# Tariq-Abuhashim/semantic-slam

Measured on AMD Instinct MI355X. Metric: Mvoxels/sec integrated, 512³ grid @ 640×480 depth; achieved HBM GB/s %peak, higher is better.
Workload: dtype f32

## Files before the change

include/tsdf_hip_diag.h:

```cpp
#ifndef TSDF_HIP_DIAG_H
#define TSDF_HIP_DIAG_H

#include "tsdf_hip.h"

#ifdef __cplusplus
extern "C" {
#endif


int tsdf_integrate_sequence_timed(tsdf_volume *vol, const float *depth_dev, const float *cam2world,
                                  int32_t n_frames, float *elapsed_ms);

int tsdf_integrate_frames_timed(tsdf_volume *vol, const float *const *depth_dev, const uint8_t *const *masks_dev,
                                const float *cam2world, int32_t n_frames, float *elapsed_ms);


int tsdf_probe_graph_replay(tsdf_volume *vol, const float *depth_dev, const float *cam2world, int32_t n_frames,
                            int32_t iters, float *ms_launches, float *ms_graph);

int tsdf_probe_stream(tsdf_volume *vol, int32_t non_temporal, int32_t n_iters, float *elapsed_ms);


int tsdf_selftest_fastdiv(int32_t device, uint64_t seed, uint64_t n_samples, float fx, float cx,
                          uint64_t *mismatches, float first_bad[4]);

int tsdf_selftest_fastdiv_band(int32_t device, uint64_t seed, uint64_t n_samples, uint64_t *mismatches,
                               float first_bad[4]);

int tsdf_selftest_round(int32_t device, uint64_t *mismatches, float first_bad[4]);

int tsdf_selftest_tile_tables(int32_t device, const float *depth_dev, const uint8_t *mask_dev, int32_t im_height,
                              int32_t im_width, float max_depth, uint64_t *mismatches);


int32_t tsdf_frames_per_launch(const tsdf_volume *vol);
int tsdf_shortcut_stats(tsdf_volume *vol, int32_t enable, uint64_t counts_out[3]);
int tsdf_brick_list_stats(tsdf_volume *vol, uint64_t counts_out[4]);
int tsdf_classification_info(tsdf_volume *vol, double info_out[2]);

int tsdf_store_stats(tsdf_volume *vol, int64_t out[9]);

int tsdf_last_cam2base(const tsdf_volume *vol, float out[16]);


int tsdf_set_kernel_variant(tsdf_volume *vol, int32_t variant);

int tsdf_set_brick_shape(tsdf_volume *vol, int32_t quads, int32_t rows, int32_t slices);
int tsdf_brick_shape(const tsdf_volume *vol, int32_t shape_out[3]);
int tsdf_default_brick_shape(const tsdf_config *cfg, int32_t shape_out[3]);

#ifdef __cplusplus
}
#endif
#endif
```

semantic_slam_amd/capi.py:

```python
import ctypes as C
import os

import numpy as np

_PKG = os.path.dirname(os.path.abspath(__file__))
LIB_PATH = os.environ.get("TSDF_HIP_LIB") or os.path.join(_PKG, "libtsdf_hip.so")

ABI_SYMBOLS = [
    "tsdf_config_default", "tsdf_create", "tsdf_destroy", "tsdf_reset", "tsdf_integrate",
    "tsdf_integrate_u16", "tsdf_convert_depth_u16", "tsdf_set_deferral",
    "tsdf_integrate_device", "tsdf_integrate_cam2base", "tsdf_integrate_masked_device",
    "tsdf_integrate_frames_device",
    "tsdf_sync", "tsdf_download", "tsdf_copy_slices", "tsdf_upload", "tsdf_refresh_summary", "tsdf_device_ptrs", "tsdf_slab_voxels", "tsdf_frames_per_launch", "tsdf_shortcut_stats", "tsdf_brick_list_stats", "tsdf_classification_info", "tsdf_store_stats",
    "tsdf_get_config", "tsdf_last_cam2base", "tsdf_set_stream", "tsdf_get_stream",
    "tsdf_count_surface", "tsdf_extract_surface", "tsdf_extract_crossings", "tsdf_extract_mesh", "tsdf_save_mesh_ply", "tsdf_save_mesh_welded_ply", "tsdf_save_ply", "tsdf_save_bin", "tsdf_load_bin", "tsdf_save_state", "tsdf_load_state",
    "tsdf_integrate_sequence_timed", "tsdf_integrate_frames_timed", "tsdf_probe_graph_replay", "tsdf_probe_stream", "tsdf_selftest_fastdiv", "tsdf_selftest_fastdiv_band", "tsdf_selftest_round", "tsdf_selftest_tile_tables", "tsdf_set_kernel_variant", "tsdf_set_brick_shape", "tsdf_brick_shape", "tsdf_default_brick_shape", "tsdf_last_error",
    "tsdf_version", "tsdf_multiply_matrix", "tsdf_invert_matrix",
    "tsdf_labels_enable", "tsdf_compose_labels", "tsdf_integrate_labels_device", "tsdf_integrate_frames_labels_device",
    "tsdf_download_labels",
    "tsdf_colour_enable", "tsdf_integrate_colour_device", "tsdf_integrate_rgbd", "tsdf_download_colour",
    "tsdf_raycast_params_default", "tsdf_raycast_device", "tsdf_raycast", "tsdf_batch_raycast_device",
    "tsdf_track_params_default", "tsdf_track", "tsdf_track_system",
    "tsdf_batch_track", "tsdf_batch_track_system", "tsdf_track_member_systems",
    "tsdf_fuse_params_default", "tsdf_fuse_volume",
    "tsdf_extent_params_default", "tsdf_volume_extent", "tsdf_batch_extents", "tsdf_group_extent", "tsdf_extent_combine",
    "tsdf_extent_metric", "tsdf_extent_regrid",
    "tsdf_associate_params_default", "tsdf_associate_count", "tsdf_associate_assign", "tsdf_batch_associate",
    "tsdf_segment_params_default", "tsdf_segmenter_create", "tsdf_segmenter_destroy", "tsdf_segmenter_set_stream",
    "tsdf_segment_depth_device", "tsdf_segment_refine_masks_device", "tsdf_segment_frame",
    "tsdf_object_origin", "tsdf_batch_create", "tsdf_batch_destroy", "tsdf_batch_size", "tsdf_batch_volume",
    "tsdf_batch_integrate_device", "tsdf_batch_sync",
    "tsdf_group_create", "tsdf_group_destroy", "tsdf_group_size", "tsdf_group_voxels", "tsdf_group_volume",
    "tsdf_group_integrate", "tsdf_group_integrate_frames", "tsdf_group_set_deferral", "tsdf_group_sync", "tsdf_group_reset", "tsdf_group_download",
    "tsdf_group_extract_surface", "tsdf_group_extract_crossings", "tsdf_group_extract_mesh",
    "tsdf_group_save_ply", "tsdf_group_save_mesh_ply", "tsdf_group_save_bin",
]
DIAG_SYMBOLS = [
    "tsdf_integrate_sequence_timed", "tsdf_integrate_frames_timed",
    "tsdf_probe_graph_replay", "tsdf_probe_stream",
    "tsdf_selftest_fastdiv", "tsdf_selftest_fastdiv_band", "tsdf_selftest_round", "tsdf_selftest_tile_tables",
    "tsdf_shortcut_stats", "tsdf_brick_list_stats", "tsdf_classification_info", "tsdf_store_stats", "tsdf_frames_per_launch", "tsdf_last_cam2base",
    "tsdf_set_kernel_variant", "tsdf_set_brick_shape", "tsdf_brick_shape", "tsdf_default_brick_shape",
]


class TsdfError(RuntimeError):
    pass


SHIPPED_VARIANTS = (0, 1, 3, 7, 8)


def experiments_build():
    return b"+experiments" in load().tsdf_version()


def variants(*wanted):
    exp = experiments_build()
    return [v for v in wanted if v in SHIPPED_VARIANTS or exp]


class TsdfConfig(C.Structure):
    _fields_ = [
        ("im_height", C.c_int32), ("im_width", C.c_int32),
# ... 108 lines not shown
    L.tsdf_integrate.argtypes = [vp, vp, vp]
    L.tsdf_set_deferral.argtypes = [vp, C.c_int32]
    L.tsdf_integrate_u16.argtypes = [vp, vp, C.c_float, C.c_int32, C.c_int32, vp]
    L.tsdf_convert_depth_u16.argtypes = [vp, vp, vp, C.c_float, C.c_int32, C.c_int32]
    L.tsdf_integrate_device.argtypes = [vp, vp, vp]
    L.tsdf_integrate_cam2base.argtypes = [vp, vp, vp]
    L.tsdf_integrate_masked_device.argtypes = [vp, vp, vp, vp]
    L.tsdf_integrate_frames_device.argtypes = [vp, vp, vp, vp, C.c_int32]
    L.tsdf_sync.argtypes = [vp]
    L.tsdf_download.argtypes = [vp, vp, vp]
    L.tsdf_upload.argtypes = [vp, vp, vp]
    L.tsdf_copy_slices.argtypes = [vp, C.c_int32, C.c_int32, vp, vp]
    L.tsdf_refresh_summary.argtypes = [vp]
    L.tsdf_device_ptrs.argtypes = [vp, C.POINTER(vp), C.POINTER(vp)]
    L.tsdf_slab_voxels.argtypes = [vp]
    L.tsdf_slab_voxels.restype = C.c_int64
    L.tsdf_frames_per_launch.argtypes = [vp]
    L.tsdf_frames_per_launch.restype = C.c_int32
    L.tsdf_shortcut_stats.argtypes = [vp, C.c_int32, vp]
    L.tsdf_classification_info.argtypes = [vp, vp]
    L.tsdf_brick_list_stats.argtypes = [vp, vp]
    if hasattr(L, "tsdf_store_stats"):
        L.tsdf_store_stats.argtypes = [vp, i64p]
    L.tsdf_get_config.argtypes = [vp, C.POINTER(TsdfConfig)]
    L.tsdf_last_cam2base.argtypes = [vp, vp]
    L.tsdf_set_stream.argtypes = [vp, vp]
    L.tsdf_get_stream.argtypes = [vp, C.POINTER(vp)]
    L.tsdf_count_surface.argtypes = [vp, C.c_float, i64p]
    L.tsdf_extract_surface.argtypes = [vp, C.c_float, vp, C.c_int64, i64p]
    L.tsdf_extract_crossings.argtypes = [vp, vp, vp, C.c_float, vp, C.c_int64, i64p]
    L.tsdf_extract_mesh.argtypes = [vp, vp, vp, C.c_float, vp, C.c_int64, i64p]
    L.tsdf_save_mesh_ply.argtypes = [vp, C.c_char_p, C.c_float]
    L.tsdf_save_mesh_welded_ply.argtypes = [vp, C.c_char_p, C.c_float]
    L.tsdf_save_ply.argtypes = [vp, C.c_char_p, C.c_float]
    L.tsdf_save_bin.argtypes = [vp, C.c_char_p]
    L.tsdf_load_bin.argtypes = [vp, C.c_char_p]
    L.tsdf_save_state.argtypes = [vp, C.c_char_p]
    L.tsdf_load_state.argtypes = [vp, C.c_char_p]
    L.tsdf_integrate_sequence_timed.argtypes = [vp, vp, vp, C.c_int32, f32p]
    L.tsdf_integrate_frames_timed.argtypes = [vp, vp, vp, vp, C.c_int32, f32p]
    L.tsdf_probe_graph_replay.argtypes = [vp, vp, vp, C.c_int32, C.c_int32, f32p, f32p]
    L.tsdf_probe_stream.argtypes = [vp, C.c_int32, C.c_int32, f32p]
    L.tsdf_selftest_fastdiv.argtypes = [C.c_int32, C.c_uint64, C.c_uint64, C.c_float, C.c_float, C.POINTER(C.c_uint64), f32p]
    L.tsdf_selftest_fastdiv_band.argtypes = [C.c_int32, C.c_uint64, C.c_uint64, C.POINTER(C.c_uint64), f32p]
    L.tsdf_selftest_round.argtypes = [C.c_int32, C.POINTER(C.c_uint64), f32p]
    L.tsdf_selftest_tile_tables.argtypes = [C.c_int32, vp, vp, C.c_int32, C.c_int32, C.c_float, C.POINTER(C.c_uint64)]
# ... 352 lines not shown
    def n_voxels(self):
        return int(self.lib.tsdf_slab_voxels(self._h))

    def shortcut_stats(self, enable=True):
        out = (C.c_uint64 * 3)()
        check(self.lib.tsdf_shortcut_stats(self._h, 1 if enable else 0, out), "tsdf_shortcut_stats")
        return tuple(int(x) for x in out)

    def brick_list_stats(self):
        out = (C.c_uint64 * 4)()
        check(self.lib.tsdf_brick_list_stats(self._h, out), "tsdf_brick_list_stats")
        return tuple(int(x) for x in out)

    def classification_info(self):
        out = (C.c_double * 2)()
        check(self.lib.tsdf_classification_info(self._h, out), "tsdf_classification_info")
        return float(out[0]), int(out[1])

    def store_stats(self):
        out = (C.c_int64 * 9)()
        check(self.lib.tsdf_store_stats(self._h, out), "tsdf_store_stats")
        return {name: tuple(int(x) for x in out[3 * k:3 * k + 3]) for k, name in enumerate(("frames", "masks", "tables"))}

    @property
    def frames_per_launch(self):
        return int(self.lib.tsdf_frames_per_launch(self._h))

    @property
    def slab_shape(self):
        c = self.cfg
        return (c.z_end - c.z_begin, c.dim_y, c.dim_x)

    def device_ptrs(self):
        t, w = C.c_void_p(), C.c_void_p()
        check(self.lib.tsdf_device_ptrs(self._h, C.byref(t), C.byref(w)), "tsdf_device_ptrs")
        return t.value, w.value

    def integrate(self, depth_host, cam2world):
        d = _f32(depth_host, self.cfg.im_height * self.cfg.im_width)
        p = _f32(cam2world, 16)
        check(self.lib.tsdf_integrate(self._h, d.ctypes.data, p.ctypes.data), "tsdf_integrate")

    def set_deferral(self, n_frames):
        check(self.lib.tsdf_set_deferral(self._h, n_frames), "tsdf_set_deferral")

    def integrate_u16(self, raw_u16, cam2world, depth_factor=5000.0, row_step=1, col_step=1):
# ... 490 lines not shown
```

semantic_slam_amd/csrc/host_derive.h:

```cpp
#pragma once
#include <algorithm>
#include <cmath>
#include <cstddef>
#include <cstdint>

#include "tsdf_hip.h"

namespace tsdf_host {

inline bool brick_shape_ok(const tsdf_config &c, int q, int r, int s)
{
    return c.dim_x % 4 == 0 && q >= 1 && r >= 1 && s >= 1 && q * r * s <= 64 && (c.dim_x / 4) % q == 0 &&
           (long long)s * c.dim_x * c.dim_y < (1ll << 30);
}

inline void choose_brick_default(const tsdf_config &c, int &bq, int &br, int &bs)
{
    bq = 0; br = 0; bs = 1;
    if (c.dim_x % 4 != 0) return;
    const int quads = c.dim_x / 4;
    const int nz = c.z_end - c.z_begin;
    double best = 1e300;
    for (int q = 1; q <= 64 && q <= quads; ++q) {
        if (quads % q) continue;
// ... 138 lines not shown
constexpr int64_t kWindowBytes = 512ll << 20;

struct SweepWindow { int cache_lo, cache_hi; };

inline SweepWindow sweep_window(int nz, int dim_x, int dim_y, int64_t window_bytes, bool reverse)
{
    const int64_t slice_bytes = 8 * (int64_t)dim_x * dim_y;
    const int w = (int)std::min<int64_t>(nz, window_bytes / slice_bytes);
    return reverse ? SweepWindow{0, w} : SweepWindow{nz - w, nz};
}

inline bool batch_defers(int members, int64_t total_voxels) { return 2 * (int64_t)members < 10 + total_voxels / 1000000; }

constexpr int64_t kBatchMinVoxelsPerMember = 2000000;
inline bool batch_classifies(Classify mode, int members, int64_t launch_voxels)
{
    const bool big_enough = mode == Classify::Always || launch_voxels >= (int64_t)members * kBatchMinVoxelsPerMember;
    return big_enough && classify_one_frame(mode, launch_voxels);
}

constexpr int kBatchSideStreams = 4;
inline int batch_lanes(int members) { return members < 8 ? 1 : kBatchSideStreams; }

struct Regions {
    size_t add(size_t bytes) { const size_t at = (end_ + 255) / 256 * 256; end_ = at + bytes; return at; }
    size_t total() const { return end_; }
    size_t end_ = 0;
};

}
```

semantic_slam_amd/csrc/tsdf_capi.hip:

```cpp
#include "../../include/tsdf_hip.h"
#include "../../include/tsdf_hip_diag.h"

#include <hip/hip_runtime.h>

#include <algorithm>
#include <cmath>
#include <cstdarg>
#include <cstdio>
#include <cstdlib>
#include <cstring>
#include <new>
#include <string>
#include <vector>

#include "pose_math.h"
#include "host_derive.h"
#include "host_copy.h"
#include "hip_owned.h"
#include "frame_store.h"
#include "tsdf_kernels.hip.h"
#include "tsdf_multiframe.hip.h"
#include "tsdf_labels.hip.h"
#include "tsdf_colour.hip.h"
#include "tsdf_extract.hip.h"
// ... 76 lines not shown
    struct tsdf_group *group_owner = nullptr;
    bool in_flush = false;
    float pend_c2b[16 * tsdfk::kMaxFramesPerLaunch] = {};
    const uint8_t *pend_mask[tsdfk::kMaxFramesPerLaunch] = {};
    int variant = 0;
    int sweep_parity = 0;
#ifdef TSDF_EXPERIMENTS
    StageRing<Staged<tsdfk::FramePose>, kStageSlots> frames;
#endif
    DevPtr<uint16_t> d_label;
    DevPtr<float> d_fp, d_bp;
    float prob_thd = 0.0f;
    DevPtr<uint32_t> d_colour;
    StageRing<Staged<uint8_t>, kStageSlots> rgb;
    DevPtr<uint32_t> d_flags;
    size_t n_flags = 0;
    int nseg = 0;
    int chunks_per_slice = 0;
    bool flat = false;
    int brick_q = 0, brick_r = 0, brick_s = 0;
    int tile = 0;
    bool fine_tables = false;
    bool flags_known_zero = false;
#ifdef TSDF_EXPERIMENTS
    DevBuf<unsigned int> d_super;
#endif
    DevBuf<uint4> d_work;
    int64_t work_nsuper = 0, work_bucket_supers = 0;
    int work_wedge_mode = -1;
    DevPtr<unsigned int> d_shortcut_stats;
    DevPtr<unsigned long long> d_claims;
    HostPtr<unsigned long long> h_claims;
    Event claims_done;
    Stream pre_stream, rb_stream;
    int rb_parity = -1;
    Event pre_done[2], list_free[2], seq_ready;
    int list_parity = 0;
    bool list_used[2] = {false, false};
    bool pipeline_ok = false;
    bool claims_pending = false, claims_known = false;
    double claims_total = 0.0;
    double claim_fraction = 0.0;
    int launches_unclassified = 0;
    DevBuf<char> d_scratch;
    DevBuf<uint8_t> d_wg_class;
    DevBuf<char> d_list;
// ... 229 lines not shown
            const int strips = ((p.tiles_w + 3) / 4) * p.tiles_h;
            hipLaunchKernelGGL(tsdfk::depth_tile_summary<16>, dim3((unsigned)((strips + 3) / 4), m), dim3(64, 4), 0, stream, tp);
        } else {
            const int strips = ((p.tiles_w + 7) / 8) * p.tiles_h;
            hipLaunchKernelGGL(tsdfk::depth_tile_summary<8>, dim3((unsigned)((strips + 3) / 4), m), dim3(64, 4), 0, stream, tp);
        }
        if (p.tiles_w * p.tiles_h <= tsdfk::kTileLdsEntries) {
            const unsigned threads = (p.tiles_w * p.tiles_h > 2048 && !beside_a_launch) ? 1024 : 256;
            const unsigned fine_blocks = fine ? ((unsigned)(p.fine_w * p.fine_h) + threads - 1) / threads : 0u;
            hipLaunchKernelGGL(tsdfk::tile_sparse_table, dim3((unsigned)tsdf_host::tile_levels(p.tiles_w) + fine_blocks, m), dim3(threads), 0, stream, tp.tiles,
                               p.tiles_w, p.tiles_h, k == 0 ? zero_me : (unsigned long long *)nullptr, fine, p.fine_w, p.fine_h);
        } else {
            if (zero_me && k == 0) HIP_TRY(hipMemsetAsync(zero_me, 0, tsdfk::kCounterBytes, stream));
            hipLaunchKernelGGL(tsdfk::tile_sparse_table_scan, dim3((unsigned)tsdf_host::tile_levels(p.tiles_w), m), dim3(256), 0, stream, tp.tiles,
                               p.tiles_w, p.tiles_h);
            if (fine)
                hipLaunchKernelGGL(tsdfk::fine_tile_levels, dim3((unsigned)((p.fine_w * p.fine_h + 255) / 256), m), dim3(256), 0, stream, fine, p.fine_w, p.fine_h);
        }
    }
    HIP_TRY(hipGetLastError());
    return TSDF_OK;
}

int launch_masked_bricks(tsdf_volume *v, tsdfk::IntegrateParams &p)
{
    const int blocks = (p.brick_groups * p.bricks_per_group + 3) / 4, nz = (p.nz + p.brick_s - 1) / p.brick_s;
    StoreSlot table;
    int rc0 = table.take(v, &v->store->tables, v->stream);
    if (rc0) return rc0;
    const size_t n_bricks = (size_t)blocks * nz * 4;
    HIP_TRY(v->d_wg_class.ensure(n_bricks));
    const float *d = p.depth;
    const uint8_t *m = p.mask;
    int rc = build_tile_tables(v->stream, v->cfg, p, &d, &m, 1, table.as<float2>());
    if (rc) return rc;
    tsdfk::FramePose pose;
    pose_from_params(pose, p);
    pose.tiles = table.as<float2>();
    hipLaunchKernelGGL(tsdfk::classify_bricks, dim3((unsigned)((n_bricks + 255) / 256)), dim3(256), 0, v->stream, p, pose,
                       v->d_wg_class, blocks, nz);
    p.wg_class = v->d_wg_class;
    hipLaunchKernelGGL((tsdfk::integrate_single_bricks<kBrickNT>), dim3(blocks, 1, nz), dim3(64, 4, 1), 0, v->stream, p, pose);
    HIP_TRY(hipGetLastError());
    return table.release();
}

int drop_summary(tsdf_volume *v)
{
    if (v->flags_known_zero || v->n_flags == 0) return TSDF_OK;
    HIP_TRY(hipMemsetAsync(v->d_flags, 0, v->n_flags * sizeof(uint32_t), v->stream));
    v->flags_known_zero = true;
    return TSDF_OK;
}

int rebuild_summary(tsdf_volume *v)
{
    if (v->n_flags == 0 || v->n_vox == 0) return TSDF_OK;
    const int nz = v->cfg.z_end - v->cfg.z_begin;
    const int qps = (int)((int64_t)v->cfg.dim_x * v->cfg.dim_y / 4);
    dim3 block(64, 4, 1), grid((v->chunks_per_slice + 3) / 4, 1, nz);
    hipLaunchKernelGGL(tsdfk::recompute_flags, grid, block, 0, v->stream, v->d_tsdf, v->d_weight, v->d_flags, qps,
                       v->chunks_per_slice);
    HIP_TRY(hipGetLastError());
    v->flags_known_zero = false;
    return TSDF_OK;
}

int launch_multi(tsdf_volume *v, const float *const *depth_dev, const uint8_t *const *masks_dev, const float *c2b, int n,
                 const uint16_t *const *label_ims = nullptr, const float *const *score_ims = nullptr, hipEvent_t inputs_ready = nullptr);

double claims_read_back(const tsdf_volume *v)
{
    double claimed = 0.0;
    for (int b = 0; b < tsdfk::kListBuckets; ++b) {
        const unsigned long long w = v->h_claims[(size_t)b * (tsdfk::kBucketStride / sizeof(unsigned long long)) + 1];
        claimed += (double)(w >> 32) + (double)(w & 0xffffffffull);
    }
    return v->claims_total > 0 ? claimed / v->claims_total : 0.0;
}

#ifdef TSDF_EXPERIMENTS
tsdf_host::Variant experiment_variant(int variant);
void experiment_adjust(const tsdf_volume *v, bool labels, bool *classify, int *z_fastest);
int launch_integrate_experiment(tsdf_volume *v, const float *depth_dev, const uint8_t *mask_dev, const float *c2b);
int launch_multi_experiment(tsdf_volume *v, tsdfk::MultiParamsInline &mi, const float *const *depth_dev, const uint8_t *const *masks_dev,
                            const float *c2b, int n, bool labels, bool any_mask, bool classify, bool *handled, double *claims_total);
bool experiment_takes_multi(const tsdf_volume *v, bool labels, bool classify);
// ... 43 lines not shown
        const tsdfk::IntegrateParams p = make_params(v, depth_dev, mask_dev, c2b, 1);
        dim3 block(64, 4, 1), grid((c.dim_x + 63) / 64, (c.dim_y + 3) / 4, nz);
        if (mask_dev) hipLaunchKernelGGL((tsdfk::integrate_scalar<true>), grid, block, 0, v->stream, p);
        else hipLaunchKernelGGL((tsdfk::integrate_scalar<false>), grid, block, 0, v->stream, p);
        HIP_TRY(hipGetLastError());
        return TSDF_OK;
    }
    if (v->flat) {
        return launch_multi(v, &depth_dev, mask_dev ? &mask_dev : nullptr, c2b, 1);
    }
    tsdfk::IntegrateParams p = make_params(v, depth_dev, mask_dev, c2b, 4);
    v->flags_known_zero = false;
    const dim3 block(64, 4, 1), grid((p.xgroups + 63) / 64, (p.dim_y + 7) / 8, p.nz);
    if (mask_dev) {
        const bool classify = tsdf_host::classify_one_frame(var.classify, v->n_vox) && tiles_fit(p.tiles_w, p.tiles_h);
        if (classify && p.brick_q > 0 && (!kExperiments || v->variant != 11)) {
            int rc = launch_masked_bricks(v, p);
            if (rc) return rc;
        } else {
#ifdef TSDF_EXPERIMENTS
            if (v->variant == 11 && classify) return launch_integrate_experiment(v, depth_dev, mask_dev, c2b);
#endif
            set_sweep(v, p);
            hipLaunchKernelGGL((tsdfk::integrate_tile<2, true>), grid, block, 0, v->stream, p);
        }
    } else {
        set_sweep(v, p);
        hipLaunchKernelGGL((tsdfk::integrate_tile<2, false>), grid, block, 0, v->stream, p);
    }
    HIP_TRY(hipGetLastError());
    return TSDF_OK;
}

void compose_cam2base(const tsdf_volume *v, const float *cam2world, float *c2b)
{
    tsdf_host::multiply_matrix(v->base2world_inv, cam2world, c2b);
}

int launch_multi(tsdf_volume *v, const float *const *depth_dev, const uint8_t *const *masks_dev,
                 const float *c2b, int n, const uint16_t *const *label_ims, const float *const *score_ims, hipEvent_t inputs_ready)
{
    const tsdf_config &c = v->cfg;
    const int nz = c.z_end - c.z_begin;
    if (nz == 0 || n == 0) return TSDF_OK;
    auto fill_pose = [&](tsdfk::FramePose &fp, int f) {
        pose_from_params(fp, make_params(v, depth_dev[f], masks_dev ? masks_dev[f] : nullptr, c2b + 16 * f, 4));
        fp.label_im = label_ims ? label_ims[f] : nullptr;
        fp.score_im = label_ims ? score_ims[f] : nullptr;
    };
    const dim3 block(64, 4, 1);
    if (n == 1 && !label_ims) {
        tsdfk::IntegrateParams common = make_params(v, depth_dev[0], nullptr, c2b, 4);
        tsdfk::FramePose pose;
        fill_pose(pose, 0);
        std::memcpy(v->last_cam2base, c2b, sizeof v->last_cam2base);
        v->flags_known_zero = false;
#ifdef TSDF_EXPERIMENTS
        {
            bool handled = false;
            int rc = launch_single_experiment(v, common, pose, depth_dev[0], c2b, &handled);
            if (rc || handled) return rc;
        }
#endif
        if (v->flat && pose.mask != nullptr && tsdf_host::classify_one_frame(variant_of(v->variant).classify, v->n_vox) &&
            tiles_fit(common.tiles_w, common.tiles_h) && common.brick_q > 0) {
            tsdfk::IntegrateParams cp = make_params(v, depth_dev[0], pose.mask, c2b, 4);
            return launch_masked_bricks(v, cp);
// ... 373 lines not shown
    rc = frame.release();
    store_next_pass(v);
    return rc;
}

int apply_host_frame(tsdf_volume *v, StoreSlot &frame, const float cam2world[16], bool defer, bool copies_marked, const uint8_t *rgb_dev = nullptr)
{
    StoreSlot no_mask;
    if (defer) return pool_slot_commit(v, frame, no_mask, cam2world);
    if (!copies_marked) HIP_TRY(hipEventRecord(v->pend_copied, v->copy_stream));
    HIP_TRY(hipStreamWaitEvent(v->stream, v->pend_copied, 0));
    return launch_staged_frame(v, frame, cam2world, rgb_dev);
}

int fill(tsdf_volume *v)
{
    if (v->n_vox == 0) return TSDF_OK;
    size_t n = (size_t)v->n_vox;
    int blocks = (int)std::min<size_t>((n / 4 + 255) / 256, 256 * 8);
    if (blocks < 1) blocks = 1;
    hipLaunchKernelGGL(tsdfk::fill_grid, dim3(blocks), dim3(256), 0, v->stream, v->d_tsdf, v->d_weight, n);
    HIP_TRY(hipGetLastError());
    if (v->n_flags) {
        HIP_TRY(hipMemsetD32Async((hipDeviceptr_t)v->d_flags, 3, v->n_flags, v->stream));
        v->flags_known_zero = false;
    }
    return TSDF_OK;
}

#ifdef TSDF_EXPERIMENTS
#include "tsdf_experiments_host.hip.h"
#endif

}

extern "C" {

const char *tsdf_last_error(void) { return g_last_error.c_str(); }

const char *tsdf_version(void)
{
    return kExperiments ? "tsdf_hip 0.3 (gfx950) +experiments" : "tsdf_hip 0.3 (gfx950)";
}

void tsdf_multiply_matrix(const float a[16], const float b[16], float out[16])
{
    tsdf_host::multiply_matrix(a, b, out);
}
// ... 657 lines not shown
    if (rc) return rc;
    HIP_TRY(hipStreamSynchronize(b->stream));
    return TSDF_OK;
}

int tsdf_batch_integrate_device(tsdf_batch *b, const float *depth_dev, const uint8_t *const *masks_dev,
                                const float cam2world[16])
{
    if (!b || !depth_dev || !cam2world) return fail(TSDF_ERR_INVALID, "tsdf_batch_integrate_device: NULL argument");
    HIP_TRY(hipSetDevice(b->device));
    if (b->total_slices == 0) return TSDF_OK;
    const int n = (int)b->vols.size();
    for (tsdf_volume *v : b->vols)
        if (v->pend_count > 0) { int rc = flush_pending(v); if (rc) return rc; }
    {
        bool defer = b->vols[0]->defer_n > 1;
        int64_t total = 0;
        for (tsdf_volume *v : b->vols) { defer = defer && can_fuse(v); total += v->n_vox; }
        defer = defer && tsdf_host::batch_defers(n, total);
        if (defer) return batch_collect(b, depth_dev, masks_dev, cam2world);
        int rc = batch_flush(b);
        if (rc) return rc;
    }
    decltype(b->blocks)::Slot *s = nullptr;
    HIP_TRY(b->blocks.take(&s));
    tsdfk::IntegrateParams *const h_params = s->params.host, *const d_params = s->params.dev;
    tsdfk::FramePose *const h_poses = s->poses.host, *const d_poses = s->poses.dev;
    for (int i = 0; i < n; ++i) {
        tsdf_volume *v = b->vols[i];
        float c2b[16];
        compose_cam2base(v, cam2world, c2b);
        std::memcpy(v->last_cam2base, c2b, sizeof c2b);
        const tsdfk::IntegrateParams q = make_params(v, depth_dev, masks_dev ? masks_dev[i] : nullptr, c2b, 4);
        h_params[i] = q;
        pose_from_params(h_poses[i], q);
        v->flags_known_zero = false;
    }
    bool any_mask = false;
    for (int i = 0; i < n && masks_dev; ++i) any_mask = any_mask || masks_dev[i] != nullptr;
    bool same_range = true;
    for (int i = 1; i < n; ++i) same_range = same_range && b->vols[i]->cfg.max_depth == b->vols[0]->cfg.max_depth;
    int64_t launch_voxels = 0;
    for (tsdf_volume *v : b->vols) launch_voxels += v->n_vox;
    const bool classify = any_mask && same_range && tsdf_host::batch_classifies(variant_of(b->vols[0]->variant).classify, n, launch_voxels) &&
                          tiles_fit(h_params[0].tiles_w, h_params[0].tiles_h);
    if (classify) {
// ... 76 lines not shown
```

semantic_slam_amd/csrc/tsdf_diag.hip.h:

```cpp
#pragma once

namespace {

template <typename Queue>
int time_on_stream(tsdf_volume *v, const char *who, float *elapsed_ms, Queue &&queue)
{
    Event e0, e1;
    HIP_TRY(event_create(e0, hipEventDefault));
    HIP_TRY(event_create(e1, hipEventDefault));
    HIP_TRY(hipEventRecord(e0, v->stream));
    const int rc = queue();
    hipError_t er = hipEventRecord(e1, v->stream);
    hipError_t es = hipEventSynchronize(e1);
    float ms = 0.f;
    hipError_t et = hipEventElapsedTime(&ms, e0, e1);
    if (rc) return rc;
    if (er != hipSuccess || es != hipSuccess || et != hipSuccess)
        return fail(TSDF_ERR_HIP, "%s: event timing failed", who);
    *elapsed_ms = ms;
    return TSDF_OK;
}

int frames_timed(tsdf_volume *v, const float *const *depth_dev, const uint8_t *const *masks_dev,
                 const float *cam2world, int32_t n_frames, float *elapsed_ms, const char *who)
// ... 281 lines not shown
    unsigned int h[8] = {0, 0, 0, 0, 0, 0, 0, 0};
    if (v->d_shortcut_stats) HIP_TRY(hipMemcpy(h, v->d_shortcut_stats, sizeof h, hipMemcpyDeviceToHost));
    for (int i = 0; i < 4; ++i) counts_out[i] = h[3 + i];
    return TSDF_OK;
}

int tsdf_classification_info(tsdf_volume *v, double info_out[2])
{
    if (!v || !info_out) return fail(TSDF_ERR_INVALID, "tsdf_classification_info: NULL argument");
    int rc = bind_device(v);
    if (rc) return rc;
    HIP_TRY(hipStreamSynchronize(v->stream));
    if (v->rb_stream) HIP_TRY(hipStreamSynchronize(v->rb_stream));
    if (v->claims_pending && hipEventQuery(v->claims_done) == hipSuccess) {
        v->claim_fraction = claims_read_back(v);
        v->claims_pending = false;
        v->claims_known = true;
    }
    info_out[0] = v->claims_known ? v->claim_fraction : -1.0;
    info_out[1] = (double)v->launches_unclassified;
    return TSDF_OK;
}

int tsdf_store_stats(tsdf_volume *v, int64_t out[9])
{
    if (!v || !out) return fail(TSDF_ERR_INVALID, "tsdf_store_stats: NULL argument");
    tsdf_store::store_counts(v->store, v, out);
    return TSDF_OK;
}

int tsdf_last_cam2base(const tsdf_volume *v, float out[16])
{
    if (!v || !out) return fail(TSDF_ERR_INVALID, "tsdf_last_cam2base: NULL argument");
    std::memcpy(out, v->last_cam2base, sizeof v->last_cam2base);
    return TSDF_OK;
}


int tsdf_set_kernel_variant(tsdf_volume *v, int32_t variant)
{
    if (!v) return fail(TSDF_ERR_INVALID, "tsdf_set_kernel_variant: NULL handle");
    if (!variant_of(variant).known)
        return fail(TSDF_ERR_INVALID, "tsdf_set_kernel_variant: unknown variant %d (this build knows 0, 1, 3, 7, 8%s)", variant,
                    kExperiments ? " and the experiments" : "; the others live in the -DTSDF_EXPERIMENTS build");
    v->variant = variant;
    return TSDF_OK;
// ... 33 lines not shown
```

semantic_slam_amd/csrc/tsdf_experiments_host.hip.h:

```cpp
#pragma once

tsdf_host::Variant experiment_variant(int variant)
{
    using tsdf_host::Classify;
    const int c = (variant - 32) & 15;
    const bool sum_ok = (variant >= 32 && variant < 112 && c < 12 && ((c >> 1) & 1)) || variant == 115 || variant == 119;
    if (variant == 2 || (variant >= 16 && variant < 28) || sum_ok) return {true, false, false, Classify::Adaptive};
    if ((variant >= 4 && variant <= 6) || variant == 9 || variant == 10) return {true, true, false, Classify::Adaptive};
    if (variant >= 11 && variant <= 13) return {true, true, false, Classify::Always};
    return {};
}

void experiment_adjust(const tsdf_volume *v, bool labels, bool *classify, int *z_fastest)
{
    if (v->variant == 9) *z_fastest = 0;
    if (v->variant == 10) *z_fastest = 1;
    if (labels && v->variant == 11) *classify = false;
}

template <int R, bool ELIDE, bool NT, bool MASKED, bool SUM, bool EARLY = false, bool FAST = false>
void launch_ladder(const tsdf_volume *v, const tsdfk::IntegrateParams &p)
{
    dim3 block(64, 4, 1);
    dim3 grid((p.xgroups + 63) / 64, (p.dim_y + 4 * R - 1) / (4 * R), p.nz);
// ... 11 lines not shown
    const uint8_t *m = p.mask;
    int rc = build_tile_tables(v->stream, v->cfg, p, &d, &m, 1, tiles);
    if (rc) return rc;
    tsdfk::FramePose pose;
    pose_from_params(pose, p);
    pose.tiles = tiles;
    hipLaunchKernelGGL(tsdfk::classify_workgroups, dim3((unsigned)((n_wg + 255) / 256)), dim3(256), 0, v->stream, p, pose,
                       v->d_wg_class, nbx, nby, nz, rows_per_wg);
    HIP_TRY(hipGetLastError());
    p.wg_class = v->d_wg_class;
    return TSDF_OK;
}


int launch_integrate_experiment(tsdf_volume *v, const float *depth_dev, const uint8_t *mask_dev, const float *c2b)
{
    const tsdf_config &c = v->cfg;
    const int nz = c.z_end - c.z_begin;
    const int variant = v->variant;
    if (v->flat && variant != 2) return launch_multi(v, &depth_dev, mask_dev ? &mask_dev : nullptr, c2b, 1);
    tsdfk::IntegrateParams p = make_params(v, depth_dev, mask_dev, c2b, 4);
    if (variant == 11) {
        v->flags_known_zero = false;
        const dim3 grid((p.xgroups + 63) / 64, (p.dim_y + 7) / 8, p.nz);
        StoreSlot table;
        int rc = classify_single(v, table, p, (int)grid.x, (int)grid.y, (int)grid.z, 8);
        if (rc) return rc;
        hipLaunchKernelGGL((tsdfk::ladder_tile<2, true, true, true, true, false, true, false, true>), grid, dim3(64, 4, 1), 0, v->stream, p);
        HIP_TRY(hipGetLastError());
        return table.release();
    }
    const bool summary = variant != 2 && ((variant >= 32 && variant < 64) || (variant >= 80 && variant < 96) || variant >= 112);
    if (!summary) {
        int rc = drop_summary(v);
        if (rc) return rc;
    } else {
        v->flags_known_zero = false;
    }
    if (variant == 2) {
        dim3 block(64, 4, 1), grid((p.xgroups + 63) / 64, (c.dim_y + 3) / 4, nz);
        if (mask_dev) hipLaunchKernelGGL((tsdfk::ladder_rows<4, true>), grid, block, 0, v->stream, p);
        else hipLaunchKernelGGL((tsdfk::ladder_rows<4, false>), grid, block, 0, v->stream, p);
    } else if (variant >= 32) {
        switch (variant - 32) {
#define SUM_CASE(code, R, N, S, E) case code: launch_ladder<R, true, N, false, S, E>(v, p); break;
#define FAST_CASE(code, R, N, S) case code: launch_ladder<R, true, N, false, S, false, true>(v, p); break;
            FAST_CASE(48 + 2, 1, false, true) FAST_CASE(48 + 3, 1, true, true)
            FAST_CASE(48 + 6, 2, false, true) FAST_CASE(48 + 7, 2, true, true)
            FAST_CASE(48 + 10, 4, false, true) FAST_CASE(48 + 11, 4, true, true)
            FAST_CASE(64 + 2, 1, false, false) FAST_CASE(64 + 3, 1, true, false)
            FAST_CASE(64 + 6, 2, false, false) FAST_CASE(64 + 7, 2, true, false)
            FAST_CASE(64 + 10, 4, false, false) FAST_CASE(64 + 11, 4, true, false)
#undef FAST_CASE
            case 80 + 3: hipLaunchKernelGGL((tsdfk::ladder_tile<1, true, true, false, true, false, true, true>),
                                            dim3((p.xgroups + 63) / 64, (p.dim_y + 3) / 4, p.nz), dim3(64, 4, 1), 0, v->stream, p); break;
            case 80 + 7: hipLaunchKernelGGL((tsdfk::ladder_tile<2, true, true, false, true, false, true, true>),
                                            dim3((p.xgroups + 63) / 64, (p.dim_y + 7) / 8, p.nz), dim3(64, 4, 1), 0, v->stream, p); break;
            SUM_CASE(2, 1, false, true, false) SUM_CASE(3, 1, true, true, false)
            SUM_CASE(6, 2, false, true, false) SUM_CASE(7, 2, true, true, false)
            SUM_CASE(10, 4, false, true, false) SUM_CASE(11, 4, true, true, false)
// ... 130 lines not shown
```

semantic_slam_amd/csrc/tsdf_kernels.hip.h:

```cpp
#pragma once
#include <hip/hip_runtime.h>
#include <stdint.h>
#include <type_traits>

namespace tsdfk {

struct IntegrateParams {
    const float *depth;
    const uint8_t *mask;
    float *tsdf;
    float *weight;
    float fx, fy, cx, cy;
    float rx0, rx1, rx2;
    float ry0, ry1, ry2;
    float rz0, rz1, rz2;
    float tx, ty, tz;
    float ox, oy, oz;
    float vs, trunc, max_depth;
    int dim_x, dim_y;
    int nz, z_begin;
    int H, W;
    int xgroups;
    uint32_t *flags;
    int nseg;
    int quads_per_row, quads_per_slice, chunks_per_slice;
    int brick_q, brick_r, brick_s, bricks_per_group, brick_groups;
// ... 133 lines not shown
}
template <bool NT>
__device__ __forceinline__ void vol_store(float *p, float4 v)
{
    if constexpr (NT) {
        v4f q = {v.x, v.y, v.z, v.w};
        __builtin_nontemporal_store(q, reinterpret_cast<v4f *>(p));
    } else {
        *reinterpret_cast<float4 *>(p) = v;
    }
}

template <bool NT>
__device__ __forceinline__ float4 vol_load_p(std::integral_constant<bool, NT>, const float *p) { return vol_load<NT>(p); }
__device__ __forceinline__ float4 vol_load_p(bool nt, const float *p) { return nt ? vol_load<true>(p) : vol_load<false>(p); }
template <bool NT>
__device__ __forceinline__ void vol_store_p(std::integral_constant<bool, NT>, float *p, float4 v) { vol_store<NT>(p, v); }
__device__ __forceinline__ void vol_store_p(bool nt, float *p, float4 v)
{
    if (nt) vol_store<true>(p, v);
    else vol_store<false>(p, v);
}

__device__ __forceinline__ float gather_f32(const float *__restrict__ base, uint32_t px)
{
    return *reinterpret_cast<const float *>(reinterpret_cast<const char *>(base) + (px << 2));
}

__device__ __forceinline__ int pixel_index24(int iv, int W, int iu)
{
    return (int)(__umul24((unsigned)iv, (unsigned)W) + (unsigned)iu);
}

template <int R, int MASKED>
__device__ __forceinline__ void integrate_tile_body(const IntegrateParams &p, const int bx, const int by, const int lz,
                                                    const bool lnt, const bool snt)
{
    const int gz = p.z_begin + lz;
    const int xg = bx * 64 + threadIdx.x;
    const int gy0 = (by * 4 + threadIdx.y) * R;
    if (xg >= p.xgroups || gy0 >= p.dim_y) return;
    const size_t row0 = ((size_t)lz * p.dim_y + gy0) * (size_t)p.dim_x + (size_t)xg * 4;
    const size_t flag0 = ((size_t)lz * p.dim_y + gy0) * (size_t)p.nseg + bx;

    uint32_t fl[R];
    float4 t4[R], w4[R];
// ... 88 lines not shown
    bool upd[R][4], rowany[R], bandr[R];
    bool any = false, band = false;
#pragma unroll
    for (int r = 0; r < R; ++r) {
        rowany[r] = false;
        bandr[r] = false;
#pragma unroll
        for (int j = 0; j < 4; ++j) {
            const float d = dval[r][j];
            const float df = d - pcz[r][j];
            diff[r][j] = df;
            const bool u = geo[r][j] & !((d <= 0.0f) | (d > p.max_depth)) & !(df <= -p.trunc);
            upd[r][j] = u;
            rowany[r] |= u;
            bandr[r] |= u & !(df >= p.trunc);
        }
        band |= bandr[r];
        any |= rowany[r];
    }
    if (__ballot(any) == 0ull) return;
    if (!any) return;

#pragma unroll
    for (int r = 0; r < R; ++r) {
        if (rowany[r]) {
            const float *wp = p.weight + row0 + (size_t)r * p.dim_x, *tp = p.tsdf + row0 + (size_t)r * p.dim_x;
            w4[r] = vol_load_p(lnt, wp);
            if (!(fl[r] & 1u)) t4[r] = vol_load_p(lnt, tp);
        }
    }
    float dist[R][4];
    if (__ballot(band) != 0ull) {
#pragma unroll
        for (int r = 0; r < R; ++r)
#pragma unroll
            for (int j = 0; j < 4; ++j) dist[r][j] = fminf(1.0f, diff[r][j] / p.trunc);
    } else {
#pragma unroll
        for (int r = 0; r < R; ++r)
#pragma unroll
            for (int j = 0; j < 4; ++j) dist[r][j] = 1.0f;
    }

    auto store_rows = [&](auto snt_c) {
    #pragma unroll
        for (int r = 0; r < R; ++r) {
            if (fl[r] == 3u && __ballot(bandr[r]) == 0ull) {
                if (rowany[r]) {
                    const float4 w = w4[r];
                    vol_store_p(snt_c, p.weight + row0 + (size_t)r * p.dim_x,
                                    make_float4(upd[r][0] ? w.x + 1.0f : w.x, upd[r][1] ? w.y + 1.0f : w.y,
                                                upd[r][2] ? w.z + 1.0f : w.z, upd[r][3] ? w.w + 1.0f : w.w));
                }
                continue;
            }
            float tv[4] = {t4[r].x, t4[r].y, t4[r].z, t4[r].w};
            float wv[4] = {w4[r].x, w4[r].y, w4[r].z, w4[r].w};
            float num[4], wn[4];
            bool need = false;
    #pragma unroll
            for (int j = 0; j < 4; ++j) {
                wn[j] = wv[j] + 1.0f;
                num[j] = tv[j] * wv[j] + dist[r][j];
                need |= upd[r][j] && !(num[j] == wn[j] && wn[j] < 3.0e38f && wn[j] > 0.0f);
            }
            float nt[4];
            if (__ballot(rowany[r] && need) != 0ull) {
    #pragma unroll
                for (int j = 0; j < 4; ++j) nt[j] = num[j] / wn[j];
            } else {
    #pragma unroll
                for (int j = 0; j < 4; ++j) nt[j] = 1.0f;
            }
            bool changed = false, notone = false;
    #pragma unroll
            for (int j = 0; j < 4; ++j) {
                const float newt = upd[r][j] ? nt[j] : tv[j];
                changed |= __float_as_uint(newt) != __float_as_uint(tv[j]);
                notone |= upd[r][j] && __float_as_uint(newt) != 0x3f800000u;
                tv[j] = newt;
                wv[j] = upd[r][j] ? wn[j] : wv[j];
            }
            if ((fl[r] & 1u) && __ballot(notone) != 0ull) {
                if (notone) p.flags[flag0 + (size_t)r * p.nseg] = fl[r] & 2u;
            }
            const bool store_t = __ballot(rowany[r] && changed) != 0ull;
            if (rowany[r]) {
                if (store_t) vol_store_p(snt_c, p.tsdf + row0 + (size_t)r * p.dim_x, make_float4(tv[0], tv[1], tv[2], tv[3]));
                vol_store_p(snt_c, p.weight + row0 + (size_t)r * p.dim_x, make_float4(wv[0], wv[1], wv[2], wv[3]));
            }
        }
    };
    if constexpr (MASKED == 1) {
        if (snt) store_rows(std::true_type{});
        else store_rows(std::false_type{});
    } else {
        store_rows(snt);
    }
}

template <int R, bool MASKED>
__global__ __launch_bounds__(256) void integrate_tile(IntegrateParams p)
{
    const int lz = p.sweep_reverse ? p.nz - 1 - (int)blockIdx.z : (int)blockIdx.z;
    const bool cached = lz >= p.cache_lo && lz < p.cache_hi;
#ifdef TSDF_EXPERIMENTS
    const bool lnt = !cached && !p.head_plain_loads;
#else
    const bool lnt = !cached;
#endif
    integrate_tile_body<R, MASKED ? 1 : 0>(p, blockIdx.x, blockIdx.y, lz, lnt, !cached);
}
// ... 89 lines not shown

template <bool NT>
__global__ __launch_bounds__(256) void stream_rmw(float *tsdf, float *weight, size_t n_quads, float one,
                                                  float zero)
{
    const size_t stride = (size_t)gridDim.x * blockDim.x;
    for (size_t q = (size_t)blockIdx.x * blockDim.x + threadIdx.x; q < n_quads; q += stride) {
        float4 t = vol_load<NT>(tsdf + 4 * q);
        float4 w = vol_load<NT>(weight + 4 * q);
        t.x *= one; t.y *= one; t.z *= one; t.w *= one;
        w.x += zero; w.y += zero; w.z += zero; w.w += zero;
        vol_store<NT>(tsdf + 4 * q, t);
        vol_store<NT>(weight + 4 * q, w);
    }
}

__global__ __launch_bounds__(256) void recompute_flags(const float *tsdf, const float *weight, uint32_t *flags,
                                                       int quads_per_slice, int chunks_per_slice)
{
    const int chunk = blockIdx.x * 4 + threadIdx.y;
    if (chunk >= chunks_per_slice) return;
    const int q = chunk * 64 + threadIdx.x;
    const size_t base = ((size_t)blockIdx.z * quads_per_slice + q) * 4;
    bool ones = true, sane = true;
    if (q < quads_per_slice) {
        const float4 t = *reinterpret_cast<const float4 *>(tsdf + base);
        const float4 w = *reinterpret_cast<const float4 *>(weight + base);
        ones = __float_as_uint(t.x) == 0x3f800000u && __float_as_uint(t.y) == 0x3f800000u &&
               __float_as_uint(t.z) == 0x3f800000u && __float_as_uint(t.w) == 0x3f800000u;
        sane = w.x >= 0.0f && w.x < 3.0e38f && w.y >= 0.0f && w.y < 3.0e38f && w.z >= 0.0f && w.z < 3.0e38f &&
               w.w >= 0.0f && w.w < 3.0e38f;
    }
    const uint32_t f = (__ballot(!ones) == 0ull ? 1u : 0u) | (__ballot(!sane) == 0ull ? 2u : 0u);
    if (threadIdx.x == 0) flags[(size_t)blockIdx.z * chunks_per_slice + chunk] = f;
}

__global__ __launch_bounds__(256) void depth_u16_to_f32(const uint16_t *raw, float *out, int H, int W,
                                                        float scale, int row_step, int col_step)
{
    const int n = H * W;
    for (int i = blockIdx.x * blockDim.x + threadIdx.x; i < n; i += gridDim.x * blockDim.x) {
        const int r = i / W, c = i - r * W;
        const bool keep = (r % row_step == 0) && (c % col_step == 0);
        out[i] = (keep ? (float)raw[i] : 0.0f) * scale;
    }
}

__device__ __forceinline__ void atomic_min_float(float *addr, float v)
{
    if (__float_as_int(v) >= 0) atomicMin(reinterpret_cast<int *>(addr), __float_as_int(v));
    else atomicMax(reinterpret_cast<unsigned int *>(addr), __float_as_uint(v));
}

__global__ __launch_bounds__(256) void object_origin(const float *depth, const uint8_t *mask, int H, int W, float fx,
                                                     float fy, float cx, float cy, float *out)
{
    float mx = 1000.0f, my = 1000.0f, mz = 1000.0f;
// ... 32 lines not shown
```

Baseline: 408,500.

## Track uniform weight runs in summary flags to skip weight loads

Extends the per-chunk summary flag word with a 'run' bit and a 24-bit count recording that every weight in the 64-quad chunk holds the same integer value. The integrate kernel then synthesises the weights from the flag instead of loading them from HBM. It increments the count when the whole chunk is updated and drops the run bit otherwise, and uses non-temporal stores for weights in run chunks. Paths that cannot maintain runs (masked bricks, multi-frame, batch, experiments) call a new kernel that clears the run bits first. A diagnostic summary_stats API is also added. The cost removed is weight-read bandwidth on uniformly weighted regions, in exchange for extra flag writes, wave-wide ballots, and the risk of weight and flag state drifting apart.

```diff
diff --git a/include/tsdf_hip_diag.h b/include/tsdf_hip_diag.h
--- a/include/tsdf_hip_diag.h
+++ b/include/tsdf_hip_diag.h
@@ -38,6 +38,8 @@
 int tsdf_brick_list_stats(tsdf_volume *vol, uint64_t counts_out[4]);
 int tsdf_classification_info(tsdf_volume *vol, double info_out[2]);
 
+int tsdf_summary_stats(tsdf_volume *vol, uint64_t out[3]);
+
 int tsdf_store_stats(tsdf_volume *vol, int64_t out[9]);
 
 int tsdf_last_cam2base(const tsdf_volume *vol, float out[16]);
diff --git a/semantic_slam_amd/capi.py b/semantic_slam_amd/capi.py
--- a/semantic_slam_amd/capi.py
+++ b/semantic_slam_amd/capi.py
@@ -11,7 +11,7 @@
     "tsdf_integrate_u16", "tsdf_convert_depth_u16", "tsdf_set_deferral",
     "tsdf_integrate_device", "tsdf_integrate_cam2base", "tsdf_integrate_masked_device",
     "tsdf_integrate_frames_device",
-    "tsdf_sync", "tsdf_download", "tsdf_copy_slices", "tsdf_upload", "tsdf_refresh_summary", "tsdf_device_ptrs", "tsdf_slab_voxels", "tsdf_frames_per_launch", "tsdf_shortcut_stats", "tsdf_brick_list_stats", "tsdf_classification_info", "tsdf_store_stats",
+    "tsdf_sync", "tsdf_download", "tsdf_copy_slices", "tsdf_upload", "tsdf_refresh_summary", "tsdf_device_ptrs", "tsdf_slab_voxels", "tsdf_frames_per_launch", "tsdf_shortcut_stats", "tsdf_brick_list_stats", "tsdf_classification_info", "tsdf_store_stats", "tsdf_summary_stats",
     "tsdf_get_config", "tsdf_last_cam2base", "tsdf_set_stream", "tsdf_get_stream",
     "tsdf_count_surface", "tsdf_extract_surface", "tsdf_extract_crossings", "tsdf_extract_mesh", "tsdf_save_mesh_ply", "tsdf_save_mesh_welded_ply", "tsdf_save_ply", "tsdf_save_bin", "tsdf_load_bin", "tsdf_save_state", "tsdf_load_state",
     "tsdf_integrate_sequence_timed", "tsdf_integrate_frames_timed", "tsdf_probe_graph_replay", "tsdf_probe_stream", "tsdf_selftest_fastdiv", "tsdf_selftest_fastdiv_band", "tsdf_selftest_round", "tsdf_selftest_tile_tables", "tsdf_set_kernel_variant", "tsdf_set_brick_shape", "tsdf_brick_shape", "tsdf_default_brick_shape", "tsdf_last_error",
@@ -39,7 +39,7 @@
     "tsdf_integrate_sequence_timed", "tsdf_integrate_frames_timed",
     "tsdf_probe_graph_replay", "tsdf_probe_stream",
     "tsdf_selftest_fastdiv", "tsdf_selftest_fastdiv_band", "tsdf_selftest_round", "tsdf_selftest_tile_tables",
-    "tsdf_shortcut_stats", "tsdf_brick_list_stats", "tsdf_classification_info", "tsdf_store_stats", "tsdf_frames_per_launch", "tsdf_last_cam2base",
+    "tsdf_shortcut_stats", "tsdf_brick_list_stats", "tsdf_classification_info", "tsdf_store_stats", "tsdf_summary_stats", "tsdf_frames_per_launch", "tsdf_last_cam2base",
     "tsdf_set_kernel_variant", "tsdf_set_brick_shape", "tsdf_brick_shape", "tsdf_default_brick_shape",
 ]
 
@@ -194,6 +194,8 @@
     L.tsdf_brick_list_stats.argtypes = [vp, vp]
     if hasattr(L, "tsdf_store_stats"):
         L.tsdf_store_stats.argtypes = [vp, i64p]
+    if hasattr(L, "tsdf_summary_stats"):
+        L.tsdf_summary_stats.argtypes = [vp, vp]
     L.tsdf_get_config.argtypes = [vp, C.POINTER(TsdfConfig)]
     L.tsdf_last_cam2base.argtypes = [vp, vp]
     L.tsdf_set_stream.argtypes = [vp, vp]
@@ -592,6 +594,11 @@
         check(self.lib.tsdf_store_stats(self._h, out), "tsdf_store_stats")
         return {name: tuple(int(x) for x in out[3 * k:3 * k + 3]) for k, name in enumerate(("frames", "masks", "tables"))}
 
+    def summary_stats(self):
+        out = (C.c_uint64 * 3)()
+        check(self.lib.tsdf_summary_stats(self._h, out), "tsdf_summary_stats")
+        return tuple(int(x) for x in out)
+
     @property
     def frames_per_launch(self):
         return int(self.lib.tsdf_frames_per_launch(self._h))
diff --git a/semantic_slam_amd/csrc/host_derive.h b/semantic_slam_amd/csrc/host_derive.h
--- a/semantic_slam_amd/csrc/host_derive.h
+++ b/semantic_slam_amd/csrc/host_derive.h
@@ -184,6 +184,35 @@
 constexpr int kBatchSideStreams = 4;
 inline int batch_lanes(int members) { return members < 8 ? 1 : kBatchSideStreams; }
 
+#if defined(__HIPCC__)
+#define TSDF_HOST_DEVICE __host__ __device__
+#else
+#define TSDF_HOST_DEVICE
+#endif
+
+constexpr uint32_t kSummaryOnes = 1u, kSummarySane = 2u, kSummaryRun = 4u;
+constexpr int kRunCountShift = 8;
+constexpr uint32_t kMaxRunCount = (1u << 24) - 1;
+constexpr uint32_t kSummaryFresh = kSummaryOnes | kSummarySane | kSummaryRun;
+
+TSDF_HOST_DEVICE inline bool word_has_run(uint32_t word) { return (word & kSummaryRun) != 0u; }
+TSDF_HOST_DEVICE inline uint32_t word_run_count(uint32_t word) { return word >> kRunCountShift; }
+TSDF_HOST_DEVICE inline uint32_t word_with_run(uint32_t low, uint32_t c)
+{
+    return (low & (kSummaryOnes | kSummarySane)) | kSummaryRun | (c << kRunCountShift);
+}
+TSDF_HOST_DEVICE inline uint32_t word_without_run(uint32_t word) { return word & (kSummaryOnes | kSummarySane); }
+
+TSDF_HOST_DEVICE inline uint32_t word_after_update(uint32_t word, bool touched, bool all_updated, bool left_not_one)
+{
+    if (!touched) return word;
+    if (left_not_one) word &= ~kSummaryOnes;
+    if (!word_has_run(word)) return word;
+    const uint32_t c = word_run_count(word);
+    if (!all_updated || c >= kMaxRunCount) return word_without_run(word);
+    return word_with_run(word, c + 1u);
+}
+
 struct Regions {
     size_t add(size_t bytes) { const size_t at = (end_ + 255) / 256 * 256; end_ = at + bytes; return at; }
     size_t total() const { return end_; }
diff --git a/semantic_slam_amd/csrc/tsdf_capi.hip b/semantic_slam_amd/csrc/tsdf_capi.hip
--- a/semantic_slam_amd/csrc/tsdf_capi.hip
+++ b/semantic_slam_amd/csrc/tsdf_capi.hip
@@ -122,6 +122,7 @@
     int tile = 0;
     bool fine_tables = false;
     bool flags_known_zero = false;
+    bool runs_maybe_set = false;
 #ifdef TSDF_EXPERIMENTS
     DevBuf<unsigned int> d_super;
 #endif
@@ -397,8 +398,20 @@
     return TSDF_OK;
 }
 
+int forget_weight_runs(tsdf_volume *v)
+{
+    if (!v->runs_maybe_set || v->n_flags == 0) return TSDF_OK;
+    const unsigned blocks = (unsigned)std::min<size_t>((v->n_flags + 255) / 256, (size_t)256 * 8);
+    hipLaunchKernelGGL(tsdfk::forget_runs, dim3(blocks), dim3(256), 0, v->stream, v->d_flags.get(), v->n_flags);
+    HIP_TRY(hipGetLastError());
+    v->runs_maybe_set = false;
+    return TSDF_OK;
+}
+
 int launch_masked_bricks(tsdf_volume *v, tsdfk::IntegrateParams &p)
 {
+    int rcf = forget_weight_runs(v);
+    if (rcf) return rcf;
     const int blocks = (p.brick_groups * p.bricks_per_group + 3) / 4, nz = (p.nz + p.brick_s - 1) / p.brick_s;
     StoreSlot table;
     int rc0 = table.take(v, &v->store->tables, v->stream);
@@ -425,6 +438,7 @@
     if (v->flags_known_zero || v->n_flags == 0) return TSDF_OK;
     HIP_TRY(hipMemsetAsync(v->d_flags, 0, v->n_flags * sizeof(uint32_t), v->stream));
     v->flags_known_zero = true;
+    v->runs_maybe_set = false;
     return TSDF_OK;
 }
 
@@ -438,6 +452,7 @@
                        v->chunks_per_slice);
     HIP_TRY(hipGetLastError());
     v->flags_known_zero = false;
+    v->runs_maybe_set = true;
     return TSDF_OK;
 }
 
@@ -527,10 +542,12 @@
             if (v->variant == 11 && classify) return launch_integrate_experiment(v, depth_dev, mask_dev, c2b);
 #endif
             set_sweep(v, p);
+            v->runs_maybe_set = true;
             hipLaunchKernelGGL((tsdfk::integrate_tile<2, true>), grid, block, 0, v->stream, p);
         }
     } else {
         set_sweep(v, p);
+        v->runs_maybe_set = true;
         hipLaunchKernelGGL((tsdfk::integrate_tile<2, false>), grid, block, 0, v->stream, p);
     }
     HIP_TRY(hipGetLastError());
@@ -548,6 +565,10 @@
     const tsdf_config &c = v->cfg;
     const int nz = c.z_end - c.z_begin;
     if (nz == 0 || n == 0) return TSDF_OK;
+    {
+        int rc = forget_weight_runs(v);
+        if (rc) return rc;
+    }
     auto fill_pose = [&](tsdfk::FramePose &fp, int f) {
         pose_from_params(fp, make_params(v, depth_dev[f], masks_dev ? masks_dev[f] : nullptr, c2b + 16 * f, 4));
         fp.label_im = label_ims ? label_ims[f] : nullptr;
@@ -967,8 +988,9 @@
     hipLaunchKernelGGL(tsdfk::fill_grid, dim3(blocks), dim3(256), 0, v->stream, v->d_tsdf, v->d_weight, n);
     HIP_TRY(hipGetLastError());
     if (v->n_flags) {
-        HIP_TRY(hipMemsetD32Async((hipDeviceptr_t)v->d_flags, 3, v->n_flags, v->stream));
+        HIP_TRY(hipMemsetD32Async((hipDeviceptr_t)v->d_flags, (int)tsdf_host::kSummaryFresh, v->n_flags, v->stream));
         v->flags_known_zero = false;
+        v->runs_maybe_set = true;
     }
     return TSDF_OK;
 }
@@ -1672,6 +1694,10 @@
         int rc = batch_flush(b);
         if (rc) return rc;
     }
+    for (tsdf_volume *v : b->vols) {
+        int rc = forget_weight_runs(v);
+        if (rc) return rc;
+    }
     decltype(b->blocks)::Slot *s = nullptr;
     HIP_TRY(b->blocks.take(&s));
     tsdfk::IntegrateParams *const h_params = s->params.host, *const d_params = s->params.dev;
diff --git a/semantic_slam_amd/csrc/tsdf_diag.hip.h b/semantic_slam_amd/csrc/tsdf_diag.hip.h
--- a/semantic_slam_amd/csrc/tsdf_diag.hip.h
+++ b/semantic_slam_amd/csrc/tsdf_diag.hip.h
@@ -327,6 +327,26 @@
     return TSDF_OK;
 }
 
+int tsdf_summary_stats(tsdf_volume *v, uint64_t out[3])
+{
+    if (!v || !out) return fail(TSDF_ERR_INVALID, "tsdf_summary_stats: NULL argument");
+    int rc = bind_device(v);
+    if (rc) return rc;
+    out[0] = out[1] = out[2] = 0;
+    if (v->n_flags == 0) { HIP_TRY(hipStreamSynchronize(v->stream)); return TSDF_OK; }
+    DevPtr<unsigned long long> d;
+    HIP_TRY(dev_alloc(d, 3 * sizeof(unsigned long long)));
+    HIP_TRY(hipMemsetAsync(d, 0, 3 * sizeof(unsigned long long), v->stream));
+    const unsigned blocks = (unsigned)std::min<size_t>((v->n_flags + 255) / 256, (size_t)256 * 8);
+    hipLaunchKernelGGL(tsdfk::summary_stats, dim3(blocks), dim3(256), 0, v->stream, (const uint32_t *)v->d_flags.get(), v->n_flags, d.get());
+    HIP_TRY(hipGetLastError());
+    unsigned long long h[3] = {0, 0, 0};
+    HIP_TRY(hipMemcpyAsync(h, d, sizeof h, hipMemcpyDeviceToHost, v->stream));
+    HIP_TRY(hipStreamSynchronize(v->stream));
+    out[0] = v->n_flags; out[1] = h[1]; out[2] = h[2];
+    return TSDF_OK;
+}
+
 int tsdf_store_stats(tsdf_volume *v, int64_t out[9])
 {
     if (!v || !out) return fail(TSDF_ERR_INVALID, "tsdf_store_stats: NULL argument");
diff --git a/semantic_slam_amd/csrc/tsdf_experiments_host.hip.h b/semantic_slam_amd/csrc/tsdf_experiments_host.hip.h
--- a/semantic_slam_amd/csrc/tsdf_experiments_host.hip.h
+++ b/semantic_slam_amd/csrc/tsdf_experiments_host.hip.h
@@ -57,6 +57,8 @@
     tsdfk::IntegrateParams p = make_params(v, depth_dev, mask_dev, c2b, 4);
     if (variant == 11) {
         v->flags_known_zero = false;
+        int rcf = forget_weight_runs(v);
+        if (rcf) return rcf;
         const dim3 grid((p.xgroups + 63) / 64, (p.dim_y + 7) / 8, p.nz);
         StoreSlot table;
         int rc = classify_single(v, table, p, (int)grid.x, (int)grid.y, (int)grid.z, 8);
@@ -71,6 +73,8 @@
         if (rc) return rc;
     } else {
         v->flags_known_zero = false;
+        int rc = forget_weight_runs(v);
+        if (rc) return rc;
     }
     if (variant == 2) {
         dim3 block(64, 4, 1), grid((p.xgroups + 63) / 64, (c.dim_y + 3) / 4, nz);
diff --git a/semantic_slam_amd/csrc/tsdf_kernels.hip.h b/semantic_slam_amd/csrc/tsdf_kernels.hip.h
--- a/semantic_slam_amd/csrc/tsdf_kernels.hip.h
+++ b/semantic_slam_amd/csrc/tsdf_kernels.hip.h
@@ -2,6 +2,8 @@
 #include <hip/hip_runtime.h>
 #include <stdint.h>
 #include <type_traits>
+
+#include "host_derive.h"
 
 namespace tsdfk {
 
@@ -181,6 +183,10 @@
     else vol_store<false>(p, v);
 }
 
+__device__ __forceinline__ std::true_type weights_nt(std::true_type, uint32_t) { return {}; }
+__device__ __forceinline__ bool weights_nt(std::false_type, uint32_t word) { return tsdf_host::word_has_run(word); }
+__device__ __forceinline__ bool weights_nt(bool nt, uint32_t word) { return nt || tsdf_host::word_has_run(word); }
+
 __device__ __forceinline__ float gather_f32(const float *__restrict__ base, uint32_t px)
 {
     return *reinterpret_cast<const float *>(reinterpret_cast<const char *>(base) + (px << 2));
@@ -315,10 +321,17 @@
     if (!any) return;
 
 #pragma unroll
+    for (int r = 0; r < R; ++r) fl[r] = __builtin_amdgcn_readfirstlane(fl[r]);
+#pragma unroll
     for (int r = 0; r < R; ++r) {
         if (rowany[r]) {
             const float *wp = p.weight + row0 + (size_t)r * p.dim_x, *tp = p.tsdf + row0 + (size_t)r * p.dim_x;
-            w4[r] = vol_load_p(lnt, wp);
+            if (tsdf_host::word_has_run(fl[r])) {
+                const float c = (float)tsdf_host::word_run_count(fl[r]);
+                w4[r] = make_float4(c, c, c, c);
+            } else {
+                w4[r] = vol_load_p(lnt, wp);
+            }
             if (!(fl[r] & 1u)) t4[r] = vol_load_p(lnt, tp);
         }
     }
@@ -338,12 +351,16 @@
     auto store_rows = [&](auto snt_c) {
     #pragma unroll
         for (int r = 0; r < R; ++r) {
-            if (fl[r] == 3u && __ballot(bandr[r]) == 0ull) {
+            const bool touched = __ballot(rowany[r]) != 0ull;
+            const bool whole = tsdf_host::word_has_run(fl[r]) && __popcll(__ballot(upd[r][0] & upd[r][1] & upd[r][2] & upd[r][3])) == 64;
+            if ((fl[r] & 3u) == 3u && __ballot(bandr[r]) == 0ull) {
                 if (rowany[r]) {
                     const float4 w = w4[r];
-                    vol_store_p(snt_c, p.weight + row0 + (size_t)r * p.dim_x,
+                    vol_store_p(weights_nt(snt_c, fl[r]), p.weight + row0 + (size_t)r * p.dim_x,
                                     make_float4(upd[r][0] ? w.x + 1.0f : w.x, upd[r][1] ? w.y + 1.0f : w.y,
                                                 upd[r][2] ? w.z + 1.0f : w.z, upd[r][3] ? w.w + 1.0f : w.w));
+                    const uint32_t word = tsdf_host::word_after_update(fl[r], touched, whole, false);
+                    if (word != fl[r]) p.flags[flag0 + (size_t)r * p.nseg] = word;
                 }
                 continue;
             }
@@ -374,13 +391,12 @@
                 tv[j] = newt;
                 wv[j] = upd[r][j] ? wn[j] : wv[j];
             }
-            if ((fl[r] & 1u) && __ballot(notone) != 0ull) {
-                if (notone) p.flags[flag0 + (size_t)r * p.nseg] = fl[r] & 2u;
-            }
+            const uint32_t word = tsdf_host::word_after_update(fl[r], touched, whole, (fl[r] & 1u) && __ballot(notone) != 0ull);
             const bool store_t = __ballot(rowany[r] && changed) != 0ull;
             if (rowany[r]) {
+                if (word != fl[r]) p.flags[flag0 + (size_t)r * p.nseg] = word;
                 if (store_t) vol_store_p(snt_c, p.tsdf + row0 + (size_t)r * p.dim_x, make_float4(tv[0], tv[1], tv[2], tv[3]));
-                vol_store_p(snt_c, p.weight + row0 + (size_t)r * p.dim_x, make_float4(wv[0], wv[1], wv[2], wv[3]));
+                vol_store_p(weights_nt(snt_c, fl[r]), p.weight + row0 + (size_t)r * p.dim_x, make_float4(wv[0], wv[1], wv[2], wv[3]));
             }
         }
     };
@@ -516,7 +532,8 @@
     if (chunk >= chunks_per_slice) return;
     const int q = chunk * 64 + threadIdx.x;
     const size_t base = ((size_t)blockIdx.z * quads_per_slice + q) * 4;
-    bool ones = true, sane = true;
+    bool ones = true, sane = true, same = true;
+    uint32_t first = 0u;
     if (q < quads_per_slice) {
         const float4 t = *reinterpret_cast<const float4 *>(tsdf + base);
         const float4 w = *reinterpret_cast<const float4 *>(weight + base);
@@ -524,9 +541,39 @@
                __float_as_uint(t.z) == 0x3f800000u && __float_as_uint(t.w) == 0x3f800000u;
         sane = w.x >= 0.0f && w.x < 3.0e38f && w.y >= 0.0f && w.y < 3.0e38f && w.z >= 0.0f && w.z < 3.0e38f &&
                w.w >= 0.0f && w.w < 3.0e38f;
-    }
-    const uint32_t f = (__ballot(!ones) == 0ull ? 1u : 0u) | (__ballot(!sane) == 0ull ? 2u : 0u);
+        first = __float_as_uint(w.x);
+        same = __float_as_uint(w.y) == first && __float_as_uint(w.z) == first && __float_as_uint(w.w) == first;
+    }
+    uint32_t f = (__ballot(!ones) == 0ull ? 1u : 0u) | (__ballot(!sane) == 0ull ? 2u : 0u);
+    const uint32_t lead = __builtin_amdgcn_readfirstlane(first);
+    same = same && (q >= quads_per_slice || first == lead);
+    if ((f & 2u) && __ballot(!same) == 0ull) {
+        const float wl = __uint_as_float(lead);
+        if (wl <= (float)tsdf_host::kMaxRunCount) {
+            const uint32_t c = (uint32_t)wl;
+            if (__float_as_uint((float)c) == lead) f = tsdf_host::word_with_run(f, c);
+        }
+    }
     if (threadIdx.x == 0) flags[(size_t)blockIdx.z * chunks_per_slice + chunk] = f;
+}
+
+__global__ __launch_bounds__(256) void forget_runs(uint32_t *flags, size_t n)
+{
+    const size_t stride = (size_t)gridDim.x * blockDim.x;
+    for (size_t i = (size_t)blockIdx.x * blockDim.x + threadIdx.x; i < n; i += stride) flags[i] &= 3u;
+}
+
+__global__ __launch_bounds__(256) void summary_stats(const uint32_t *flags, size_t n, unsigned long long *out)
+{
+    const size_t stride = (size_t)gridDim.x * blockDim.x;
+    unsigned int ones = 0, runs = 0;
+    for (size_t i = (size_t)blockIdx.x * blockDim.x + threadIdx.x; i < n; i += stride) {
+        const uint32_t w = flags[i];
+        ones += w & 1u;
+        runs += (w >> 2) & 1u;
+    }
+    for (int off = 32; off > 0; off >>= 1) { ones += __shfl_down(ones, off); runs += __shfl_down(runs, off); }
+    if ((threadIdx.x & 63) == 0) { atomicAdd(out + 1, (unsigned long long)ones); atomicAdd(out + 2, (unsigned long long)runs); }
 }
 
 __global__ __launch_bounds__(256) void depth_u16_to_f32(const uint16_t *raw, float *out, int H, int W,
```

Result: faster. 470,000 (median of 6 runs) (+15.0%).
